# kaist-cvml/3d-vlm-gd

Measured on AMD Instinct MI355X. Metric: image-pairs/sec (518^2, ViT-B/14 LoRA) student distillation step, higher is better.
Workload: dtype tf32h; 1 GPU; finetune_timm_mast3r_objaverse: vit_base/14 + LoRA(r=4,q,v)+adapters blocks 4-11, 518^2 pairs, shared-518 geometry, mast3r losses (AP+depth+intra+cost-KL), 32 pairs/GPU, 300 keypoints/pair, hw=1369; pairs_per_gpu=32, global_pairs=32, parallelism=dp1, world_size_seen=1, backend=nccl (RCCL), exchange=torch, engine_dtype=tf32h

## Files before the change

3d-vlm-gd_amd/csrc/cabi.hip:

```cpp
#include "gd_common.h"
#include <stdarg.h>
#include <stdio.h>
#include <stdlib.h>
#include <string.h>

static thread_local char g_err[512] = "";

void gd_set_error(const char* fmt, ...) {
    va_list ap;
    va_start(ap, fmt);
    vsnprintf(g_err, sizeof(g_err), fmt, ap);
    va_end(ap);
}

extern "C" const char* gd_last_error(void) { return g_err; }

struct KnobDef { const char* name; const char* env; int GdKnobs::*field; int def; };
static const KnobDef KNOBS[] = {
    {"gemm_persist", "GD_GEMM_PERSIST", &GdKnobs::gemm_persist, 1},       {"gemm_small_tiles", "GD_GEMM_SMALL_TILES", &GdKnobs::gemm_small_tiles, 0},
    {"gemm_f32_big", "GD_GEMM_F32_BIG", &GdKnobs::gemm_f32_big, 0},       {"gemm_cstore", "GD_GEMM_CSTORE", &GdKnobs::gemm_cstore, 1},
    {"gemm_anat", "GD_GEMM_ANAT", &GdKnobs::gemm_anat, 0},                {"gemm_batch_big_m", "GD_GEMM_BATCH_BIG_M", &GdKnobs::gemm_batch_big_m, 384},
    {"gemm_krot", "GD_GEMM_KROT", &GdKnobs::gemm_krot, 1},                {"tn_blocks", "GD_TN_BLOCKS", &GdKnobs::tn_blocks, 0},
    {"attn_dma", "GD_ATTN_DMA", &GdKnobs::attn_dma, 1},                   {"attn_rot", "GD_ATTN_ROT", &GdKnobs::attn_rot, 1},
    {"attn_dq_dma", "GD_ATTN_DQ_DMA", &GdKnobs::attn_dq_dma, 1},
    {"attn_dkv_dma", "GD_ATTN_DKV_DMA", &GdKnobs::attn_dkv_dma, 1},
    {"attn_dkv_nw", "GD_ATTN_DKV_NW", &GdKnobs::attn_dkv_nw, 0},          {"cv_mask_skip", "GD_CV_MASK_SKIP", &GdKnobs::cv_mask_skip, 1},
    {"cv_persist", "GD_CV_PERSIST", &GdKnobs::cv_persist, 1},             {"cv_dbg", "GD_CV_DBG", &GdKnobs::cv_dbg, 0},
    {"cv_grid", "GD_CV_GRID", &GdKnobs::cv_grid, 0},                      {"pair_rank_wave", "GD_PAIR_RANK_WAVE", &GdKnobs::pair_rank_wave, 0},
    {"ln_16b", "GD_LN_16B", &GdKnobs::ln_16b, 1},                         {"adapter_persist", "GD_ADAPTER_PERSIST", &GdKnobs::adapter_persist, 1},
    {"reserve_cus", "GD_RESERVE_CUS", &GdKnobs::reserve_cus, 0},          {"gemm_group_m", "GD_GEMM_GROUP_M", &GdKnobs::gemm_group_m, 1},
};
static void gd_apply_reserve(GdKnobs& v) {
    int r = v.reserve_cus < 0 ? 0 : v.reserve_cus;
    if (r > v.ncu_dev - 8) r = v.ncu_dev - 8;
    v.ncu = v.ncu_dev - (r > 0 ? r : 0);
}

GdKnobs& gd_knobs_mut() {
    static GdKnobs k = [] {
        GdKnobs v = {};
        for (const KnobDef& d : KNOBS) {
            const char* e = getenv(d.env);
            v.*(d.field) = e ? atoi(e) : d.def;
        }
        v.ncu_dev = 256;
        int dev = 0, cus = 0;
        if (hipGetDevice(&dev) == hipSuccess && hipDeviceGetAttribute(&cus, hipDeviceAttributeMultiprocessorCount, dev) == hipSuccess && cus > 0)
            v.ncu_dev = cus;
        gd_apply_reserve(v);
        return v;
    }();
    return k;
}

extern "C" int gd_debug_set(const char* name, int value) {
    GD_REQUIRE(name != nullptr, "gd_debug_set: null name");
    for (const KnobDef& d : KNOBS)
        if (strcmp(d.name, name) == 0) { gd_knobs_mut().*(d.field) = value; gd_apply_reserve(gd_knobs_mut()); return 0; }
    gd_set_error("gd_debug_set: unknown option '%s'", name);
    return -1;
}
extern "C" int gd_debug_get(const char* name) {
    if (name)
        for (const KnobDef& d : KNOBS)
            if (strcmp(d.name, name) == 0) return gd_knobs().*(d.field);
    gd_set_error("gd_debug_get: unknown option '%s'", name ? name : "(null)");
    return -1;
}
extern "C" int gd_abi_version(void) { return GD_ABI_VERSION; }
```

3d-vlm-gd_amd/csrc/gd_knobs.h:

```cpp
#pragma once

struct GdKnobs {
    int gemm_persist;
    int gemm_small_tiles;
    int gemm_f32_big;
    int gemm_cstore;
    int gemm_group_m;
    int gemm_krot;
    int gemm_batch_big_m;
    int gemm_anat;
    int tn_blocks;
    int attn_dma;
    int attn_rot;
    int attn_dq_dma;
    int attn_dkv_dma;
    int attn_dkv_nw;
    int cv_mask_skip;
    int cv_persist;
    int cv_dbg;
    int cv_grid;
    int pair_rank_wave;
    int ln_16b;
    int adapter_persist;
    int reserve_cus;
    int ncu_dev;
    int ncu;
};
GdKnobs& gd_knobs_mut();
static inline const GdKnobs& gd_knobs() { return gd_knobs_mut(); }
```

3d-vlm-gd_amd/csrc/lora.hip:

```cpp
#include "gd_common.h"

struct LoraBwdParams {
    const void* X; long ldx;
    const float* t;
    const void* bt;
    float* dt;
    float* gbt;
    int M, K;
    const float* t_mul; const float* out_mul;
    int dt_scaled;
    float dt_mul;
};

#define LB_ROWS 64
#define LB_SLAB 256
#define LB_ROWB (LB_SLAB * 2 + 16)

__device__ __forceinline__ bf16x8 lb_tr_frag(const char* tile, int col0, int u, int lane) {
    typedef __attribute__((ext_vector_type(4))) short s16x4;
    typedef __attribute__((ext_vector_type(8))) short s16x8;
    const int g = lane >> 4, i = lane & 15, q = i >> 2, pp = i & 3;
    const char* a0 = tile + (32 * u + 4 * g + q) * LB_ROWB + (col0 + 4 * pp) * 2;
    const s16x4 x = __builtin_amdgcn_ds_read_tr16_b64_v4i16((__attribute__((address_space(3))) s16x4*)a0);
    const s16x4 y = __builtin_amdgcn_ds_read_tr16_b64_v4i16((__attribute__((address_space(3))) s16x4*)(a0 + 16 * LB_ROWB));
    const s16x8 z = {x[0], x[1], x[2], x[3], y[0], y[1], y[2], y[3]};
    return __builtin_bit_cast(bf16x8, z);
}

template <typename T, int NSLAB>
__global__ __launch_bounds__(256) __attribute__((amdgpu_waves_per_eu(2, 2))) void lora_bwd_fused_kernel(LoraBwdParams p) {
    typedef typename Mma<T>::Frag Frag;
    constexpr int SXB = LB_ROWS * LB_ROWB, SBB = 8 * NSLAB * LB_SLAB * 2, STB = LB_ROWS * 8 * 4;
    static_assert(SXB + SBB + STB >= 8 * NSLAB * LB_SLAB * 4, "the fp32 partial fits");
    __shared__ __attribute__((aligned(16))) char smem_lb[SXB + SBB + STB];
    char* const sX = smem_lb;
    T* const sBt = (T*)(smem_lb + SXB);
    float* const sT = (float*)(smem_lb + SXB + SBB);
    const int tid = threadIdx.x, lane = tid & 63, wave = tid >> 6, g = lane >> 4, c = lane & 15;
    const int K = p.K;
    const T* X = (const T*)p.X;
    const float tmul = p.t_mul ? *p.t_mul : 1.0f, omul = p.out_mul ? *p.out_mul : 1.0f;
    const float dtmul = p.dt_mul * (p.dt_scaled ? 1.0f : omul);
    const bool want_dt = p.bt != nullptr;
    if (want_dt)
        for (int i = tid; i < 8 * K / 8; i += 256) *(uint4*)(sBt + i * 8) = *(const uint4*)((const T*)p.bt + i * 8);

    f32x4 gacc[NSLAB][4];
#pragma unroll
    for (int s = 0; s < NSLAB; ++s)
#pragma unroll
        for (int j = 0; j < 4; ++j) gacc[s][j] = f32x4{0.f, 0.f, 0.f, 0.f};

    const int nchunk = (p.M + LB_ROWS - 1) / LB_ROWS;
    uint4 rx[8];
    auto gload = [&](int chunk, int s) {
#pragma unroll
        for (int i = 0; i < 8; ++i) {
            const int ch = tid + 256 * i, rr = ch >> 5, cc = ch & 31;
            const int m = chunk * LB_ROWS + rr;
            rx[i] = m < p.M ? *(const uint4*)(X + (long)m * p.ldx + s * LB_SLAB + cc * 8) : make_uint4(0, 0, 0, 0);
        }
    };
    int chunk = blockIdx.x;
    if (chunk < nchunk) gload(chunk, 0);
    for (; chunk < nchunk; chunk += gridDim.x) {
        f32x4 dacc = {0.f, 0.f, 0.f, 0.f};
        Frag thi[2], tlo[2];
#pragma unroll
        for (int s = 0; s < NSLAB; ++s) {
            __syncthreads();
#pragma unroll
            for (int i = 0; i < 8; ++i) {
                const int ch = tid + 256 * i, rr = ch >> 5, cc = ch & 31;
                *(uint4*)(sX + rr * LB_ROWB + cc * 16) = rx[i];
            }
            if (s == 0) {
                for (int i = tid; i < LB_ROWS * 8; i += 256) {
                    const int m = chunk * LB_ROWS + (i >> 3);
                    sT[i] = m < p.M ? p.t[(long)m * 8 + (i & 7)] : 0.f;
                }
            }
            __syncthreads();
            if (s + 1 < NSLAB) gload(chunk, s + 1);
            else if (chunk + (int)gridDim.x < nchunk) gload(chunk + gridDim.x, 0);
            if (s == 0) {
#pragma unroll
                for (int u = 0; u < 2; ++u)
#pragma unroll
                    for (int e = 0; e < 8; ++e) {
                        const int row = 32 * u + (e < 4 ? 4 * g + e : 16 + 4 * g + (e - 4));
                        const float v = c < 8 ? sT[row * 8 + c] * tmul : 0.f;
                        const T h = from_f32<T>(v);
                        thi[u][e] = h;
                        tlo[u][e] = from_f32<T>(v - to_f32<T>(h));
                    }
            }
            if (want_dt)
#pragma unroll
            for (int kc = 0; kc < LB_SLAB / 32; ++kc) {
                const Frag a = *(const Frag*)(sX + (16 * wave + c) * LB_ROWB + (32 * kc + 8 * g) * 2);
                Frag b = {};
                if (c < 8) b = *(const Frag*)(sBt + (long)c * K + s * LB_SLAB + 32 * kc + 8 * g);
                dacc = Mma<T>::mma(a, b, dacc);
            }
#pragma unroll
            for (int u = 0; u < 2; ++u)
#pragma unroll
                for (int nt = 0; nt < 4; ++nt) {
                    const Frag b = __builtin_bit_cast(Frag, lb_tr_frag(sX, 64 * wave + 16 * nt, u, lane));
                    gacc[s][nt] = Mma<T>::mma(thi[u], b, gacc[s][nt]);
                    gacc[s][nt] = Mma<T>::mma(tlo[u], b, gacc[s][nt]);
                }
        }
        if (c < 8 && want_dt) {
#pragma unroll
            for (int r = 0; r < 4; ++r) {
                const int m = chunk * LB_ROWS + 16 * wave + 4 * g + r;
                if (m < p.M) p.dt[(long)m * 8 + c] = dacc[r] * dtmul;
            }
        }
    }
    __syncthreads();
    float* red = (float*)smem_lb;
    if (g < 2) {
#pragma unroll
        for (int s = 0; s < NSLAB; ++s)
#pragma unroll
            for (int nt = 0; nt < 4; ++nt)
#pragma unroll
                for (int r = 0; r < 4; ++r) red[(4 * g + r) * K + s * LB_SLAB + 64 * wave + 16 * nt + c] = gacc[s][nt][r];
    }
    __syncthreads();
    for (int i = tid; i < 8 * K; i += 256) atomicAdd(p.gbt + i, red[i] * omul);
}

template <typename T>
static int lora_bwd_launch(const LoraBwdParams& p, hipStream_t s) {
    const int nchunk = (p.M + LB_ROWS - 1) / LB_ROWS;
    const int grid = nchunk < 512 ? nchunk : 512;
    switch (p.K / LB_SLAB) {
        case 1: hipLaunchKernelGGL((lora_bwd_fused_kernel<T, 1>), dim3(grid), dim3(256), 0, s, p); break;
        case 2: hipLaunchKernelGGL((lora_bwd_fused_kernel<T, 2>), dim3(grid), dim3(256), 0, s, p); break;
        case 3: hipLaunchKernelGGL((lora_bwd_fused_kernel<T, 3>), dim3(grid), dim3(256), 0, s, p); break;
        case 4: hipLaunchKernelGGL((lora_bwd_fused_kernel<T, 4>), dim3(grid), dim3(256), 0, s, p); break;
        case 6: hipLaunchKernelGGL((lora_bwd_fused_kernel<T, 6>), dim3(grid), dim3(256), 0, s, p); break;
        case 8: hipLaunchKernelGGL((lora_bwd_fused_kernel<T, 8>), dim3(grid), dim3(256), 0, s, p); break;
        default: gd_set_error("gd_lora_bwd_fused: K / 256 = %d not instantiated (1, 2, 3, 4, 6, 8)", p.K / LB_SLAB); return -1;
    }
    GD_LAUNCH_OK();
    return 0;
}

extern "C" int gd_lora_bwd_fused(const void* dqv, long ldx, const float* t, const void* bt, float* dt, float* gbt, int M, int K,
                                 void* stream) {
    GD_REQUIRE(M > 0 && K > 0 && K % LB_SLAB == 0 && K / LB_SLAB <= 8 && ldx % 8 == 0, "gd_lora_bwd_fused: K must be a multiple of 256 (<= 2048), ldx of 8");
    GD_REQUIRE(((uintptr_t)dqv & 15) == 0 && ((uintptr_t)bt & 15) == 0 && t && gbt && (dt || !bt), "gd_lora_bwd_fused: alignment / null pointers");
    LoraBwdParams p = {dqv, ldx, t, bt, dt, gbt, M, K, nullptr, nullptr, 0, 1.0f};
    return lora_bwd_launch<bf16>(p, (hipStream_t)stream);
}

extern "C" int gd_lora_bwd_fused_scaled(const void* dqv, long ldx, const float* t, const void* bt, float* dt, float* gbt, int M, int K, int dtype,
                                        const float* t_mul_dev, const float* out_mul_dev, int dt_scaled, float dt_mul, void* stream) {
    GD_REQUIRE(M > 0 && K > 0 && K % LB_SLAB == 0 && K / LB_SLAB <= 8 && ldx % 8 == 0, "gd_lora_bwd_fused_scaled: K must be a multiple of 256 (<= 2048), ldx of 8");
    GD_REQUIRE(((uintptr_t)dqv & 15) == 0 && ((uintptr_t)bt & 15) == 0 && t && gbt && (dt || !bt), "gd_lora_bwd_fused_scaled: alignment / null pointers");
    GD_REQUIRE(dtype == GD_BF16 || dtype == GD_F16, "gd_lora_bwd_fused_scaled: operands are bf16 or fp16 (dtype %d)", dtype);
    { int e; GD_REQUIRE(dt_mul > 0.f && dt_mul <= 1.0f && frexpf(dt_mul, &e) == 0.5f,
                        "gd_lora_bwd_fused_scaled: dt_mul = %g is not a power of two in (0, 1] (it undoes bt's shift exactly)", (double)dt_mul); }
    LoraBwdParams p = {dqv, ldx, t, bt, dt, gbt, M, K, t_mul_dev, out_mul_dev, dt_scaled, dt_mul};
    return dtype == GD_F16 ? lora_bwd_launch<f16>(p, (hipStream_t)stream) : lora_bwd_launch<bf16>(p, (hipStream_t)stream);
}
```

Before: 544.4 image-pairs/s.

## Add DMA-pipelined LoRA backward kernel with LDS ring buffer and swizzled reads

Adds a new LoRA backward kernel that streams X slabs and t rows into a multi-slot LDS ring using global_load_lds DMA. It overlaps the next slabs' loads with MFMA work, using explicit vmcnt waits and XOR-swizzled LDS layouts read via ds_read_b128 and transposed ds_read_b64_tr_b16. The grid is one block per CU (waves_per_eu 1) instead of up to 512 blocks, which cuts the number of atomic reductions into gbt. The new path is on by default. It risks lower occupancy and carries hand-written inline-asm synchronization that could be fragile.

```diff
diff --git a/3d-vlm-gd_amd/csrc/cabi.hip b/3d-vlm-gd_amd/csrc/cabi.hip
--- a/3d-vlm-gd_amd/csrc/cabi.hip
+++ b/3d-vlm-gd_amd/csrc/cabi.hip
@@ -28,6 +28,7 @@
     {"cv_persist", "GD_CV_PERSIST", &GdKnobs::cv_persist, 1},             {"cv_dbg", "GD_CV_DBG", &GdKnobs::cv_dbg, 0},
     {"cv_grid", "GD_CV_GRID", &GdKnobs::cv_grid, 0},                      {"pair_rank_wave", "GD_PAIR_RANK_WAVE", &GdKnobs::pair_rank_wave, 0},
     {"ln_16b", "GD_LN_16B", &GdKnobs::ln_16b, 1},                         {"adapter_persist", "GD_ADAPTER_PERSIST", &GdKnobs::adapter_persist, 1},
+    {"lora_dma", "GD_LORA_DMA", &GdKnobs::lora_dma, 1},                   {"lora_grid", "GD_LORA_GRID", &GdKnobs::lora_grid, 0},
     {"reserve_cus", "GD_RESERVE_CUS", &GdKnobs::reserve_cus, 0},          {"gemm_group_m", "GD_GEMM_GROUP_M", &GdKnobs::gemm_group_m, 1},
 };
 static void gd_apply_reserve(GdKnobs& v) {
diff --git a/3d-vlm-gd_amd/csrc/gd_knobs.h b/3d-vlm-gd_amd/csrc/gd_knobs.h
--- a/3d-vlm-gd_amd/csrc/gd_knobs.h
+++ b/3d-vlm-gd_amd/csrc/gd_knobs.h
@@ -21,6 +21,8 @@
     int cv_grid;
     int pair_rank_wave;
     int ln_16b;
+    int lora_dma;
+    int lora_grid;
     int adapter_persist;
     int reserve_cus;
     int ncu_dev;
diff --git a/3d-vlm-gd_amd/csrc/lora.hip b/3d-vlm-gd_amd/csrc/lora.hip
--- a/3d-vlm-gd_amd/csrc/lora.hip
+++ b/3d-vlm-gd_amd/csrc/lora.hip
@@ -1,4 +1,5 @@
 #include "gd_common.h"
+#include <type_traits>
 
 struct LoraBwdParams {
     const void* X; long ldx;
@@ -134,10 +135,219 @@
     for (int i = tid; i < 8 * K; i += 256) atomicAdd(p.gbt + i, red[i] * omul);
 }
 
+#define LB_SLABB (LB_ROWS * LB_SLAB * 2)
+#define LBD_R128(dst, addr, imm) asm volatile("ds_read_b128 %0, %1 offset:%2" : "=v"(dst) : "v"(addr), "i"(imm))
+#define LBD_TR64(dst, addr, imm) asm volatile("ds_read_b64_tr_b16 %0, %1 offset:%2" : "=v"(dst) : "v"(addr), "i"(imm))
+#define LBD_R32(dst, addr, imm) asm volatile("ds_read_b32 %0, %1 offset:%2" : "=v"(dst) : "v"(addr), "i"(imm))
+#define LBD_DMA(src, dst, nbytes)                                                                         \
+    __builtin_amdgcn_global_load_lds((const __attribute__((address_space(1))) void*)(src),               \
+                                     (__attribute__((address_space(3))) void*)(dst), nbytes, 0, 0)
+__device__ __forceinline__ int lbd_sw(int row) { return ((row & 7) << 1) | ((row >> 2) & 1); }
+template <int I, int N, typename F> __device__ __forceinline__ void lbd_static_for(F&& f) {
+    if constexpr (I < N) { f(std::integral_constant<int, I>{}); lbd_static_for<I + 1, N>(f); }
+}
+template <int N> __device__ __forceinline__ void lbd_wait_vm() { asm volatile("s_waitcnt vmcnt(%0)" ::"n"(N) : "memory"); }
+
+template <typename T, int NSLAB>
+__global__ __launch_bounds__(256) __attribute__((amdgpu_waves_per_eu(1, 1))) void lora_bwd_dma_kernel(LoraBwdParams p) {
+    typedef typename Mma<T>::Frag Frag;
+    typedef __attribute__((ext_vector_type(2))) unsigned u32x2;
+    constexpr int K = NSLAB * LB_SLAB;
+    constexpr int RING = NSLAB <= 6 ? 4 : 3;
+    constexpr int TRING = NSLAB >= 3 ? 2 : 4;
+    constexpr int STB = LB_ROWS * 8 * 4, T_OFF = RING * LB_SLABB, B_OFF = T_OFF + TRING * STB, SBB = 8 * K * 2;
+    static_assert(RING * LB_SLABB >= 8 * K * 4, "the fp32 partial fits in the ring");
+    static_assert(B_OFF + SBB <= 160 * 1024, "LDS of one CU");
+    __shared__ __attribute__((aligned(16))) char smem_lbd[B_OFF + SBB];
+    const int tid = threadIdx.x, lane = tid & 63, g = lane >> 4, c = lane & 15;
+    const int wave = __builtin_amdgcn_readfirstlane(tid >> 6);
+    const int M = p.M, G = gridDim.x;
+    const float tmul = p.t_mul ? *p.t_mul : 1.0f, omul = p.out_mul ? *p.out_mul : 1.0f;
+    const float dtmul = p.dt_mul * (p.dt_scaled ? 1.0f : omul);
+    const bool want_dt = p.bt != nullptr;
+    const long ldb = p.ldx * 2;
+    const int nchunk = (M + LB_ROWS - 1) / LB_ROWS;
+
+    const int ph = lane >> 5, pp = lane & 31;
+    long voff[8];
+    int coff[8];
+#pragma unroll
+    for (int i = 0; i < 8; ++i) {
+        const int row = 16 * wave + 2 * i + ph;
+        coff[i] = (pp ^ lbd_sw(row)) * 16;
+        voff[i] = row * ldb + coff[i];
+    }
+    auto issue = [&](int chunk, int s, int slot, int tslot) {
+        const char* xs = (const char*)p.X + s * (LB_SLAB * 2);
+        char* dst = smem_lbd + slot * LB_SLABB + wave * 8192;
+        if (chunk * LB_ROWS + LB_ROWS <= M) {
+            const char* xc = xs + (long)chunk * LB_ROWS * ldb;
+#pragma unroll
+            for (int i = 0; i < 8; ++i) LBD_DMA(xc + voff[i], dst + i * 1024, 16);
+        } else {
+#pragma unroll
+            for (int i = 0; i < 8; ++i) {
+                const int m = min(chunk * LB_ROWS + 16 * wave + 2 * i + ph, M - 1);
+                LBD_DMA(xs + m * ldb + coff[i], dst + i * 1024, 16);
+            }
+        }
+        if (s == 0) {
+#pragma unroll
+            for (int i = 0; i < 2; ++i) {
+                const long b = min((long)chunk * STB + wave * 512 + i * 256 + lane * 4, (long)M * 32 - 4);
+                LBD_DMA((const char*)p.t + b, smem_lbd + T_OFF + tslot * STB + wave * 512 + i * 256, 4);
+            }
+        }
+    };
+    if (want_dt) {
+        constexpr int CPR = K / 8;
+#pragma unroll
+        for (int i = 0; i < NSLAB; ++i) {
+            const int piece = wave * NSLAB + i, lin = piece * 64 + lane, r = lin / CPR, pos = lin % CPR;
+            LBD_DMA((const char*)p.bt + (r * CPR + (pos ^ (2 * r))) * 16, smem_lbd + B_OFF + piece * 1024, 16);
+        }
+    }
+#pragma unroll
+    for (int d = 0; d < RING - 1; ++d) {
+        const int cd = blockIdx.x + G * (d / NSLAB);
+        if (cd < nchunk) issue(cd, d % NSLAB, d, (d / NSLAB) & (TRING - 1));
+    }
+
+    const unsigned lds0 = (unsigned)(uintptr_t)(__attribute__((address_space(3))) const void*)smem_lbd;
+    unsigned aaddr[4], baddr[4], taddr[4];
+    const int tq = c >> 2, tp = c & 3;
+#pragma unroll
+    for (int j = 0; j < 4; ++j) {
+        aaddr[j] = (16 * wave + c) * 512 + (((4 * j + g) ^ lbd_sw(c)) * 16);
+        baddr[j] = lds0 + B_OFF + (c & 7) * (K * 2) + (((4 * j + g) ^ (2 * (c & 7))) * 16);
+        taddr[j] = (4 * g + tq) * 512 + (((8 * wave + 2 * j + (tp >> 1)) ^ lbd_sw(4 * g + tq)) * 16) + 8 * (tp & 1);
+    }
+    const unsigned tbase = lds0 + T_OFF + (4 * g * 8 + (c & 7)) * 4;
+
+    f32x4 gacc[NSLAB][4];
+#pragma unroll
+    for (int s = 0; s < NSLAB; ++s)
+#pragma unroll
+        for (int j = 0; j < 4; ++j) gacc[s][j] = f32x4{0.f, 0.f, 0.f, 0.f};
+
+    int slot = 0, k = 0;
+    for (int chunk = blockIdx.x; chunk < nchunk; chunk += G, ++k) {
+        f32x4 dacc = {0.f, 0.f, 0.f, 0.f};
+        Frag thi[2], tlo[2];
+        lbd_static_for<0, NSLAB>([&](auto s_c) __attribute__((always_inline)) {
+            constexpr int s = decltype(s_c)::value;
+            constexpr int I1 = (s + 1) % NSLAB == 0 ? 10 : 8, I2 = (s + 2) % NSLAB == 0 ? 10 : 8;
+            const bool e1 = chunk + G * ((s + 1) / NSLAB) < nchunk, e2 = chunk + G * ((s + 2) / NSLAB) < nchunk;
+            if (RING == 4 && e2) lbd_wait_vm<I1 + I2>();
+            else if (e1) lbd_wait_vm<I1>();
+            else lbd_wait_vm<0>();
+            __builtin_amdgcn_s_barrier();
+            asm volatile("" ::: "memory");
+            {
+                constexpr int D = RING - 1;
+                const int cn = chunk + G * ((s + D) / NSLAB);
+                if (cn < nchunk) issue(cn, (s + D) % NSLAB, slot == 0 ? RING - 1 : slot - 1, (k + (s + D) / NSLAB) & (TRING - 1));
+            }
+            const unsigned sb = lds0 + slot * LB_SLABB;
+            if (s == 0) {
+                const unsigned ta = tbase + (k & (TRING - 1)) * STB;
+                float tv[16];
+#pragma unroll
+                for (int u = 0; u < 2; ++u)
+#pragma unroll
+                    for (int e = 0; e < 8; ++e) LBD_R32(tv[8 * u + e], ta, (32 * u + (e < 4 ? e : 12 + e)) * 32);
+                asm volatile("s_waitcnt lgkmcnt(0)" : "+v"(tv[0]), "+v"(tv[1]), "+v"(tv[2]), "+v"(tv[3]), "+v"(tv[4]), "+v"(tv[5]), "+v"(tv[6]), "+v"(tv[7]),
+                             "+v"(tv[8]), "+v"(tv[9]), "+v"(tv[10]), "+v"(tv[11]), "+v"(tv[12]), "+v"(tv[13]), "+v"(tv[14]), "+v"(tv[15]));
+#pragma unroll
+                for (int u = 0; u < 2; ++u)
+#pragma unroll
+                    for (int e = 0; e < 8; ++e) {
+                        const int row = 32 * u + (e < 4 ? 4 * g + e : 16 + 4 * g + (e - 4));
+                        const float v = (c < 8 && chunk * LB_ROWS + row < M) ? tv[8 * u + e] * tmul : 0.f;
+                        const T h = from_f32<T>(v);
+                        thi[u][e] = h;
+                        tlo[u][e] = from_f32<T>(v - to_f32<T>(h));
+                    }
+            }
+            f32x4 av[8], bv[8];
+            u32x2 tr[2][4][2];
+            if (want_dt) {
+#pragma unroll
+                for (int kc = 0; kc < 8; ++kc) {
+                    LBD_R128(av[kc], sb + aaddr[kc & 3], (kc >> 2) * 256);
+                    LBD_R128(bv[kc], baddr[kc & 3], s * 512 + (kc >> 2) * 256);
+                }
+            }
+#pragma unroll
+            for (int u = 0; u < 2; ++u)
+#pragma unroll
+                for (int nt = 0; nt < 4; ++nt) {
+                    LBD_TR64(tr[u][nt][0], sb + taddr[nt], u * 16384);
+                    LBD_TR64(tr[u][nt][1], sb + taddr[nt], u * 16384 + 8192);
+                }
+            if (want_dt) {
+                asm volatile("s_waitcnt lgkmcnt(0)" : "+v"(av[0]), "+v"(av[1]), "+v"(av[2]), "+v"(av[3]), "+v"(av[4]), "+v"(av[5]), "+v"(av[6]), "+v"(av[7]),
+                             "+v"(bv[0]), "+v"(bv[1]), "+v"(bv[2]), "+v"(bv[3]), "+v"(bv[4]), "+v"(bv[5]), "+v"(bv[6]), "+v"(bv[7]));
+#pragma unroll
+                for (int kc = 0; kc < 8; ++kc) dacc = Mma<T>::mma(__builtin_bit_cast(Frag, av[kc]), __builtin_bit_cast(Frag, bv[kc]), dacc);
+                if (s == NSLAB - 1 && c < 8) {
+#pragma unroll
+                    for (int r = 0; r < 4; ++r) {
+                        const int m = chunk * LB_ROWS + 16 * wave + 4 * g + r;
+                        if (m < M) p.dt[(long)m * 8 + c] = dacc[r] * dtmul;
+                    }
+                }
+            }
+            asm volatile("s_waitcnt lgkmcnt(0)" : "+v"(tr[0][0][0]), "+v"(tr[0][0][1]), "+v"(tr[0][1][0]), "+v"(tr[0][1][1]), "+v"(tr[0][2][0]), "+v"(tr[0][2][1]),
+                         "+v"(tr[0][3][0]), "+v"(tr[0][3][1]), "+v"(tr[1][0][0]), "+v"(tr[1][0][1]), "+v"(tr[1][1][0]), "+v"(tr[1][1][1]), "+v"(tr[1][2][0]),
+                         "+v"(tr[1][2][1]), "+v"(tr[1][3][0]), "+v"(tr[1][3][1]));
+#pragma unroll
+            for (int u = 0; u < 2; ++u)
+#pragma unroll
+                for (int nt = 0; nt < 4; ++nt) {
+                    typedef __attribute__((ext_vector_type(4))) unsigned u32x4;
+                    const u32x4 z = {tr[u][nt][0][0], tr[u][nt][0][1], tr[u][nt][1][0], tr[u][nt][1][1]};
+                    const Frag b = __builtin_bit_cast(Frag, z);
+                    gacc[s][nt] = Mma<T>::mma(thi[u], b, gacc[s][nt]);
+                    gacc[s][nt] = Mma<T>::mma(tlo[u], b, gacc[s][nt]);
+                }
+            slot = slot + 1 == RING ? 0 : slot + 1;
+        });
+    }
+    lbd_wait_vm<0>();
+    __syncthreads();
+    float* red = (float*)smem_lbd;
+    if (g < 2) {
+#pragma unroll
+        for (int s = 0; s < NSLAB; ++s)
+#pragma unroll
+            for (int nt = 0; nt < 4; ++nt)
+#pragma unroll
+                for (int r = 0; r < 4; ++r) red[(4 * g + r) * K + s * LB_SLAB + 64 * wave + 16 * nt + c] = gacc[s][nt][r];
+    }
+    __syncthreads();
+    for (int i = tid; i < 8 * K; i += 256) atomicAdd(p.gbt + i, red[i] * omul);
+}
+
 template <typename T>
 static int lora_bwd_launch(const LoraBwdParams& p, hipStream_t s) {
     const int nchunk = (p.M + LB_ROWS - 1) / LB_ROWS;
-    const int grid = nchunk < 512 ? nchunk : 512;
+    const GdKnobs& kn = gd_knobs();
+    if (kn.lora_dma) {
+        const int grid = kn.lora_grid > 0 ? kn.lora_grid : (nchunk < kn.ncu ? nchunk : kn.ncu);
+        switch (p.K / LB_SLAB) {
+            case 1: hipLaunchKernelGGL((lora_bwd_dma_kernel<T, 1>), dim3(grid), dim3(256), 0, s, p); break;
+            case 2: hipLaunchKernelGGL((lora_bwd_dma_kernel<T, 2>), dim3(grid), dim3(256), 0, s, p); break;
+            case 3: hipLaunchKernelGGL((lora_bwd_dma_kernel<T, 3>), dim3(grid), dim3(256), 0, s, p); break;
+            case 4: hipLaunchKernelGGL((lora_bwd_dma_kernel<T, 4>), dim3(grid), dim3(256), 0, s, p); break;
+            case 6: hipLaunchKernelGGL((lora_bwd_dma_kernel<T, 6>), dim3(grid), dim3(256), 0, s, p); break;
+            case 8: hipLaunchKernelGGL((lora_bwd_dma_kernel<T, 8>), dim3(grid), dim3(256), 0, s, p); break;
+            default: gd_set_error("gd_lora_bwd_fused: K / 256 = %d not instantiated (1, 2, 3, 4, 6, 8)", p.K / LB_SLAB); return -1;
+        }
+        GD_LAUNCH_OK();
+        return 0;
+    }
+    const int grid = kn.lora_grid > 0 ? kn.lora_grid : (nchunk < 512 ? nchunk : 512);
     switch (p.K / LB_SLAB) {
         case 1: hipLaunchKernelGGL((lora_bwd_fused_kernel<T, 1>), dim3(grid), dim3(256), 0, s, p); break;
         case 2: hipLaunchKernelGGL((lora_bwd_fused_kernel<T, 2>), dim3(grid), dim3(256), 0, s, p); break;
```

Result: no change. 545.4 image-pairs/s, median of 5 (+0.2%).
